# martinruenz/co-fusion

Measured on AMD Instinct MI355X. Metric: frames/sec at 640x480 (N active models) + ICP-reduce achieved HBM GB/s vs peak, higher is better.
Workload: dtype f32

## Files before the change

### co_fusion_amd/csrc/surf_boot_dev.h

```cpp
#pragma once
#include "surf_batch_dev.h"

namespace cf {

__global__ void __launch_bounds__(kB) bilateral_kernel(const float* __restrict__ depth, int cols, int rows, float maxD,
                                                       float* __restrict__ out)
{
    const int i = blockIdx.x * kB + threadIdx.x;
    if (i >= cols * rows) return;
    const int y = i / cols, x = i - y * cols;
    const float value = depth[i];
    if (value > maxD || value < 0.3f) { out[i] = 0; return; }
    float sum1 = 0, sum2 = 0;
#pragma unroll
    for (int dy = -6; dy <= 6; ++dy) {
        const int cy = y + dy;
        if (cy < 0 || cy >= rows) continue;
        const float* __restrict__ rowp = depth + cy * cols + x;
#pragma unroll
        for (int dx = -6; dx <= 6; ++dx) {
            const int cx = x + dx;
            if (cx < 0 || cx >= cols) continue;
            const float tmp = rowp[dx];
            const float space2 = (float)(dx * dx + dy * dy);
            const float color2 = (value - tmp) * (value - tmp);
            const float weight = det_expf(-(space2 * 0.024691358f + color2 * 555.556f));
            sum1 += tmp * weight;
            sum2 += weight;
        }
    }
    out[i] = sum1 / sum2;
}

__global__ void __launch_bounds__(kB) feedback_kernel(const uchar4* __restrict__ rgba, const float* __restrict__ depth, int cols, int rows,
                                                      float cx, float cy, float inv_fx, float inv_fy, const float* __restrict__ tcx,
                                                      const float* __restrict__ tcy, int time, float maxDepth,
                                                      float4* __restrict__ rec , unsigned* __restrict__ flags)
{
    const int q = blockIdx.x * kB + threadIdx.x;
    if (q >= cols * rows) return;
    const int j = q / cols, i = q - j * cols;
    const int rank = i * rows + j;
    const float x = tcx[i] * (float)cols, y = tcy[j] * (float)rows;
    const f3 p = get_vertex(depth, cols, rows, i, j, x, y, cx, cy, inv_fx, inv_fy);
    if (p.z <= 0 || p.z > maxDepth) { flags[rank] = 0; return; }
    const f3 n = get_normal_central(p, depth, cols, rows, i, j, x, y, cx, cy, inv_fx, inv_fy);
    const uchar4 c = rgba[q];
    flags[rank] = 1;
    rec[rank * 3 + 0] = make_float4(p.x, p.y, p.z, confidence(x, y, cx, cy, 1.0f));
    rec[rank * 3 + 1] = make_float4(encode_color((float)c.x / 255.0f, (float)c.y / 255.0f, (float)c.z / 255.0f), 0.f, (float)c.z / 255.0f, (float)time);
    rec[rank * 3 + 2] = make_float4(n.x, n.y, n.z, get_radius(p.z, n.z, inv_fx, inv_fy));
}


__global__ void __launch_bounds__(kB) init_kernel(const float4* __restrict__ raw, const float4* __restrict__ filt,
                                                  const unsigned* __restrict__ raw_count, float4* __restrict__ out)
{
    const unsigned k = blockIdx.x * kB + threadIdx.x;
    if (k >= *raw_count) return;
    const float4 c = raw[k * 3 + 1];
    out[k * 3] = raw[k * 3];
    out[k * 3 + 1] = make_float4(c.x, 0.f, 1.f, c.w);
    out[k * 3 + 2] = filt[k * 3 + 2];
}

void launch_bilateral(hipStream_t s, const float* depth, int cols, int rows, float maxD, float* out)
{
    bilateral_kernel<<<gridFor((long long)cols * rows), kB, 0, s>>>(depth, cols, rows, maxD, out);
}
void launch_feedback(hipStream_t s, const uint8_t* rgba, const float* depth, int cols, int rows, cf_cam cam, float inv_fx, float inv_fy,
                     const float* tcx, const float* tcy, int time, float maxDepth, float* rec, unsigned* flags)
{
    feedback_kernel<<<gridFor((long long)cols * rows), kB, 0, s>>>(reinterpret_cast<const uchar4*>(rgba), depth, cols, rows, cam.cx, cam.cy, inv_fx,
                                                                   inv_fy, tcx, tcy, time, maxDepth, reinterpret_cast<float4*>(rec), flags);
}
void launch_init(hipStream_t s, const float* raw, const float* filt, const unsigned* raw_count, long long max_n, float* out)
{
    init_kernel<<<gridFor(max_n), kB, 0, s>>>(reinterpret_cast<const float4*>(raw), reinterpret_cast<const float4*>(filt), raw_count,
                                              reinterpret_cast<float4*>(out));
}

}
```

Before: 947.6.

## Tile bilateral filter through LDS with halo and interior fast path

The 13x13 bilateral filter now runs on 2D tiles. Each workgroup stages its tile plus a 6-pixel halo into shared memory, with a padded row stride to avoid bank conflicts. Interior tiles take a template path without bounds tests, and register rotation of rows plus an occupancy hint are added. This replaces 169 scattered global reads per pixel with LDS reads, at the cost of shared memory use and a 2D launch shape.

New measurement: 933.3. 1.5% lower.

```diff
diff --git a/co_fusion_amd/csrc/surf_boot_dev.h b/co_fusion_amd/csrc/surf_boot_dev.h
--- a/co_fusion_amd/csrc/surf_boot_dev.h
+++ b/co_fusion_amd/csrc/surf_boot_dev.h
@@ -3,33 +3,80 @@
 
 namespace cf {
 
-__global__ void __launch_bounds__(kB) bilateral_kernel(const float* __restrict__ depth, int cols, int rows, float maxD,
-                                                       float* __restrict__ out)
+#ifndef CF_BILATERAL_TW
+#define CF_BILATERAL_TW 32
+#endif
+constexpr int kBilR = 6;
+constexpr int kBilTW = CF_BILATERAL_TW, kBilTH = kB / kBilTW;
+constexpr int kBilSW = kBilTW + 2 * kBilR, kBilSH = kBilTH + 2 * kBilR;
+constexpr int kBilRounds = (kBilSW * kBilSH + kB - 1) / kB;
+constexpr int kBilStride = kBilSW % 32 == 28 ? kBilSW + 20 : kBilSW;
+constexpr int kBilLds = ((kBilRounds * kB - 1) / kBilSW + 1) * kBilStride;
+static_assert(kBilTW * kBilTH == kB && kBilTW >= 16, "the tile is one workgroup of whole rows");
+
+__device__ __forceinline__ void bilateral_tap(float value, float tmp, float space, float& sum1, float& sum2)
 {
-    const int i = blockIdx.x * kB + threadIdx.x;
-    if (i >= cols * rows) return;
-    const int y = i / cols, x = i - y * cols;
-    const float value = depth[i];
+    const float color2 = (value - tmp) * (value - tmp);
+    const float weight = det_expf(-(space + color2 * 555.556f));
+    sum1 += tmp * weight;
+    sum2 += weight;
+}
+
+template <bool kTested>
+__device__ __forceinline__ float bilateral_window(const float* c, float value, int x, int y, int cols, int rows)
+{
+    float sum1 = 0, sum2 = 0;
+    float t[2 * kBilR + 1], next[2 * kBilR + 1];
+#pragma unroll
+    for (int k = 0; k <= 2 * kBilR; ++k) next[k] = c[-kBilR * kBilStride + k - kBilR];
+#pragma unroll
+    for (int dy = -kBilR; dy <= kBilR; ++dy) {
+        const bool row_in = !kTested || (unsigned)(y + dy) < (unsigned)rows;
+#pragma unroll
+        for (int k = 0; k <= 2 * kBilR; ++k) {
+            t[k] = next[k];
+            if (dy < kBilR) next[k] = c[(dy + 1) * kBilStride + k - kBilR];
+        }
+#pragma unroll
+        for (int dx = -kBilR; dx <= kBilR; ++dx) {
+            const bool in = !kTested || (row_in && (unsigned)(x + dx) < (unsigned)cols);
+            float s1 = sum1, s2 = sum2;
+            bilateral_tap(value, t[dx + kBilR], (float)(dx * dx + dy * dy) * 0.024691358f, s1, s2);
+            sum1 = in ? s1 : sum1;
+            sum2 = in ? s2 : sum2;
+        }
+        asm volatile("" : "+v"(sum1), "+v"(sum2)::"memory");
+    }
+    return sum1 / sum2;
+}
+
+__global__ void __launch_bounds__(kB) __attribute__((amdgpu_waves_per_eu(5))) bilateral_kernel(const float* __restrict__ depth, int cols, int rows,
+                                                                                               int tiles_x, float maxD, float* __restrict__ out)
+{
+    __shared__ float tile[kBilLds];
+    const int by = blockIdx.x / tiles_x, bx = blockIdx.x - by * tiles_x;
+    const int x0 = bx * kBilTW, y0 = by * kBilTH;
+    float v[kBilRounds];
+    int at[kBilRounds];
+#pragma unroll
+    for (int k = 0; k < kBilRounds; ++k) {
+        const int e = k * kB + (int)threadIdx.x, r = e / kBilSW, c = e - r * kBilSW;
+        at[k] = r * kBilStride + c;
+        v[k] = depth[iclamp(y0 - kBilR + r, 0, rows - 1) * cols + iclamp(x0 - kBilR + c, 0, cols - 1)];
+    }
+#pragma unroll
+    for (int k = 0; k < kBilRounds; ++k) tile[at[k]] = v[k];
+    __syncthreads();
+    const int ty = (int)threadIdx.x / kBilTW, tx = (int)threadIdx.x - ty * kBilTW;
+    const int x = x0 + tx, y = y0 + ty;
+    if (x >= cols || y >= rows) return;
+    const float* c = tile + (ty + kBilR) * kBilStride + tx + kBilR;
+    const float value = c[0];
+    const int i = y * cols + x;
     if (value > maxD || value < 0.3f) { out[i] = 0; return; }
-    float sum1 = 0, sum2 = 0;
-#pragma unroll
-    for (int dy = -6; dy <= 6; ++dy) {
-        const int cy = y + dy;
-        if (cy < 0 || cy >= rows) continue;
-        const float* __restrict__ rowp = depth + cy * cols + x;
-#pragma unroll
-        for (int dx = -6; dx <= 6; ++dx) {
-            const int cx = x + dx;
-            if (cx < 0 || cx >= cols) continue;
-            const float tmp = rowp[dx];
-            const float space2 = (float)(dx * dx + dy * dy);
-            const float color2 = (value - tmp) * (value - tmp);
-            const float weight = det_expf(-(space2 * 0.024691358f + color2 * 555.556f));
-            sum1 += tmp * weight;
-            sum2 += weight;
-        }
-    }
-    out[i] = sum1 / sum2;
+    const bool interior = x0 >= kBilR && y0 >= kBilR && x0 + kBilTW + kBilR <= cols && y0 + kBilTH + kBilR <= rows;
+    if (interior) out[i] = bilateral_window<false>(c, value, x, y, cols, rows);
+    else out[i] = bilateral_window<true>(c, value, x, y, cols, rows);
 }
 
 __global__ void __launch_bounds__(kB) feedback_kernel(const uchar4* __restrict__ rgba, const float* __restrict__ depth, int cols, int rows,
@@ -66,7 +113,8 @@
 
 void launch_bilateral(hipStream_t s, const float* depth, int cols, int rows, float maxD, float* out)
 {
-    bilateral_kernel<<<gridFor((long long)cols * rows), kB, 0, s>>>(depth, cols, rows, maxD, out);
+    const int tiles_x = gridFor(cols, kBilTW), tiles_y = gridFor(rows, kBilTH);
+    bilateral_kernel<<<tiles_x * tiles_y, kB, 0, s>>>(depth, cols, rows, tiles_x, maxD, out);
 }
 void launch_feedback(hipStream_t s, const uint8_t* rgba, const float* depth, int cols, int rows, cf_cam cam, float inv_fx, float inv_fy,
                      const float* tcx, const float* tcy, int time, float maxDepth, float* rec, unsigned* flags)
```
